# dogeplusplus/torch-actor-critic

Measured on AMD Instinct MI355X. Metric: sac_updates_per_sec, higher is better.
Workload: dtype bf16; 1 GPU; model=SAC-MLP[256, 256]-HalfCheetah-v4, global_batch=64, seq_len=1, parallelism=dp1, obs_dim=17, act_dim=6, replay_buffer=1000000, update_window=50, graph=True, engine=fused, mode=full

## Files before the change

### torch_actor_critic_amd/algo/act.py

```python

import numpy as np
import torch


class ActKernel:

    def __init__(self, actor, obs_dim: int, act_dim: int,
                 device: torch.device, philox_seed: int = 0):
        from ..models.mlp import Actor as MlpActor
        from ..ops import require_extension
        if type(actor) is not MlpActor:
            raise TypeError("ActKernel needs the plain MLP Actor")
        if any(l.out_features > 256 for l in actor.layers) or act_dim > 64:
            raise ValueError("shape outside act-kernel limits")
        self.ext = require_extension()
        self.ws = [l.weight for l in actor.layers]
        self.bs = [l.bias for l in actor.layers]
        self.wmu = actor.mu_layer.weight
        self.bmu = actor.mu_layer.bias
        self.wls = actor.log_std_layer.weight
        self.bls = actor.log_std_layer.bias
        self.act_limit = float(actor.act_limit)
        self.lo = float(actor.log_min_std)
        self.hi = float(actor.log_max_std)
        self.seed = philox_seed ^ 0x5ACB
        self.ctr = torch.zeros(1, dtype=torch.int64, device=device)
        self.obs_in = torch.zeros(obs_dim, device=device)
        self.obs_pin = torch.zeros(obs_dim, pin_memory=True)
        self.act_out = torch.zeros(act_dim, device=device)
        self.act_pin = torch.zeros(act_dim, pin_memory=True)
        self.flag_pin = torch.zeros(1, dtype=torch.int32, pin_memory=True)
        self.flag_np = self.flag_pin.numpy()
        self.ev = torch.cuda.Event()
        import os
        self._pinned_ok = os.environ.get("TAC_AMD_ACT_PINNED", "1") != "0"
        self._handle = self.ext.act_prepare(
            self.obs_pin, self.ws, self.bs, self.wmu, self.bmu, self.wls,
            self.bls, self.act_out, self.act_pin, self.flag_pin, self.ctr,
            self.seed, self.act_limit, self.lo, self.hi)

    def act(self, state: np.ndarray) -> np.ndarray:
        self.obs_pin.copy_(torch.from_numpy(np.asarray(state,
                                                       dtype=np.float32)))
        if self._pinned_ok:
            self.flag_pin[0] = 0
            self.ext.act_fire(self._handle)
            fl = self.flag_np
            for _ in range(2_000_000):
                if fl[0] != 0:
                    return self.act_pin.numpy().copy()
            torch.cuda.synchronize()
            if fl[0] != 0:
                return self.act_pin.numpy().copy()
            self._pinned_ok = False
        self.obs_in.copy_(self.obs_pin, non_blocking=True)
        self.ext.act_step(self.obs_in, self.ws, self.bs, self.wmu,
                          self.bmu, self.wls, self.bls, self.act_out,
                          self.ctr, self.seed, self.act_limit, self.lo,
                          self.hi)
        self.act_pin.copy_(self.act_out, non_blocking=True)
        self.ev.record()
        self.ev.synchronize()
        return self.act_pin.numpy().copy()


def make_act_path(actor, obs_dim, act_dim, device, philox_seed: int = 0):
    try:
        return ActKernel(actor, obs_dim, act_dim, device, philox_seed)
    except Exception:
        return ActGraph(actor, obs_dim, act_dim, device)


class BatchedActKernel:

    path = "kernel"
    MAX_LAYERS = 4
    MAX_OBS = 512

    def __init__(self, actor, obs_dim: int, act_dim: int, max_rows: int,
                 device: torch.device, philox_seed: int = 0):
        from ..models.mlp import Actor as MlpActor
        from ..ops import require_extension
        if type(actor) is not MlpActor:
            raise TypeError("BatchedActKernel needs the plain MLP Actor")
        if (any(l.out_features > 256 for l in actor.layers)
                or not 1 <= len(actor.layers) <= self.MAX_LAYERS
                or act_dim > 64 or obs_dim > self.MAX_OBS):
            raise ValueError("shape outside act-kernel limits")
        if torch.device(device).type != "cuda":
            raise ValueError("BatchedActKernel needs a cuda device")
        if max_rows < 1:
            raise ValueError("max_rows must be >= 1")
        self.ext = require_extension()
        self.actor = actor
        self.obs_dim = int(obs_dim)
        self.act_dim = int(act_dim)
        self.max_rows = int(max_rows)
        self.act_limit = float(actor.act_limit)
        self.lo = float(actor.log_min_std)
        self.hi = float(actor.log_max_std)
        self.seed = philox_seed ^ 0xE7A1
        self.ctr = 0
        self.obs_in = torch.zeros(max_rows, obs_dim, device=device)
        self.obs_pin = torch.zeros(max_rows, obs_dim, pin_memory=True)
        self.act_out = torch.zeros(max_rows, act_dim, device=device)
        self.act_pin = torch.zeros(max_rows, act_dim, pin_memory=True)
        self.ev = torch.cuda.Event()

    def launch(self, n: int, deterministic: bool, ctr: int):
        a = self.actor
        self.ext.act_batch(
            self.obs_in, [l.weight for l in a.layers],
            [l.bias for l in a.layers], a.mu_layer.weight, a.mu_layer.bias,
            a.log_std_layer.weight, a.log_std_layer.bias, self.act_out,
            n, bool(deterministic), int(ctr), self.seed, self.act_limit,
            self.lo, self.hi)

    def act(self, states, deterministic: bool = True) -> np.ndarray:
        s = np.asarray(states, dtype=np.float32).reshape(-1, self.obs_dim)
        n = s.shape[0]
        if not 1 <= n <= self.max_rows:
            raise ValueError(f"{n} states for max_rows={self.max_rows}")
        self.obs_pin[:n].copy_(torch.from_numpy(s))
        self.obs_in[:n].copy_(self.obs_pin[:n], non_blocking=True)
        if not deterministic:
            self.ctr += 1
# ... 172 lines not shown
```

### torch_actor_critic_amd/ops/csrc/fused.hip

```cpp

#include <hip/hip_runtime.h>
#include <hip/hip_bf16.h>

#include <torch/extension.h>
#include <c10/hip/HIPStream.h>

#include <algorithm>
#include <utility>
#include <vector>

#include "replay_draw.h"

namespace fused {

using namespace replay;

using f32x4 = __attribute__((ext_vector_type(4))) float;
using bf16x8 = __attribute__((ext_vector_type(8))) __bf16;

__global__ __launch_bounds__(256)
void philox_words2_kernel(int64_t* __restrict__ out, uint64_t seed,
                          uint64_t chi, uint64_t clo0, int64_t n) {
  philox_words_row(out, seed, chi, clo0, n);
}


struct MProb {
  const float* x; const float* w; const float* bias; float* y;
  const float* mask;
  const float* x2; const float* w2; const float* mask2;
  const float* r1_col;
  const float* r1_row;
};

constexpr int MAXZ = 4;

struct MGemm {
  MProb p[MAXZ];
  int M, N, K, lda, ldy;
  int K2;
  int nz, k_chunk;
  float* part;
};

constexpr int TB = 64;
constexpr int BKB2 = 64;
constexpr int BKF2 = 16;
constexpr int LDSB2 = 72;
constexpr int LDSF2 = 17;
constexpr int BKP = 128;
constexpr int LDSP = 136;

template <bool BF16, bool MASK>
DEVINL void stage_tile(void* lds, const float* src, const float* mask,
                       int r0, int k0, int R, int C, int ld) {
  const int tid = threadIdx.x;
  const int row = tid & 63;
  if constexpr (BF16) {
    __bf16* d = (__bf16*)lds;
    const int c0 = (tid >> 6) * 16;
    const int gr = r0 + row;
    bool interior = (r0 + 64 <= R) && (k0 + 64 <= C) && ((ld & 3) == 0)
                    && ((k0 & 3) == 0);
    if (interior) {
      const float* p = src + (int64_t)gr * ld + k0 + c0;
      float v[16];
#pragma unroll
      for (int q = 0; q < 4; ++q) {
        float4 f = *(const float4*)(p + q * 4);
        v[q * 4 + 0] = f.x; v[q * 4 + 1] = f.y;
        v[q * 4 + 2] = f.z; v[q * 4 + 3] = f.w;
      }
      if constexpr (MASK) {
        const float* mp = mask + (int64_t)gr * ld + k0 + c0;
#pragma unroll
        for (int q = 0; q < 4; ++q) {
          float4 f = *(const float4*)(mp + q * 4);
          v[q * 4 + 0] = f.x > 0.f ? v[q * 4 + 0] : 0.f;
          v[q * 4 + 1] = f.y > 0.f ? v[q * 4 + 1] : 0.f;
          v[q * 4 + 2] = f.z > 0.f ? v[q * 4 + 2] : 0.f;
          v[q * 4 + 3] = f.w > 0.f ? v[q * 4 + 3] : 0.f;
        }
      }
      union { __bf16 h[16]; uint4 u[2]; } pk;
#pragma unroll
      for (int e = 0; e < 16; ++e) pk.h[e] = (__bf16)v[e];
      uint4* dst = (uint4*)&d[row * LDSB2 + c0];
      dst[0] = pk.u[0];
      dst[1] = pk.u[1];
    } else {
#pragma unroll
      for (int e = 0; e < 16; ++e) {
        int c = c0 + e;
// ... 1803 lines not shown
      dy2_1[idx] = dqs[1][i] * wt3_1[j];
    }
  }
}


constexpr int ACT_MAXL = 4;
constexpr int ACT_MAXW = 512;

struct ActArgs {
  const float* x;
  const float* w[ACT_MAXL];
  const float* b[ACT_MAXL];
  int width[ACT_MAXL];
  int n_layers, O, A;
  const float* wmu; const float* bmu;
  const float* wls; const float* bls;
  float* action;
  int64_t* ctr;
  uint64_t seed;
  float act_limit, lo, hi;
};

struct ActPinned {
  float* out_host;
  int* flag_host;
};

__global__ __launch_bounds__(256)
void act_kernel(ActArgs a, ActPinned hp) {
  __shared__ __attribute__((aligned(16))) float buf[2][ACT_MAXW];
  __shared__ unsigned long long ctr_s;
  const int tid = threadIdx.x;
  if (tid == 0) ctr_s = (unsigned long long)(++a.ctr[0]);
  for (int k = tid; k < a.O; k += blockDim.x) buf[0][k] = a.x[k];
  __syncthreads();

  int cur = 0, K = a.O;
  for (int L = 0; L < a.n_layers; ++L) {
    const int H = a.width[L];
    float acc = 0.f;
    if (tid < H) {
      acc = a.b[L][tid];
      const float* wr = a.w[L] + (int64_t)tid * K;
      int k = 0;
      for (; k + 4 <= K; k += 4) {
        acc += wr[k] * buf[cur][k] + wr[k+1] * buf[cur][k+1]
             + wr[k+2] * buf[cur][k+2] + wr[k+3] * buf[cur][k+3];
      }
      for (; k < K; ++k) acc += wr[k] * buf[cur][k];
    }
    __syncthreads();
    if (tid < H) buf[1 - cur][tid] = fmaxf(acc, 0.f);
    __syncthreads();
    cur ^= 1;
    K = H;
  }

  if (tid < a.A) {
    float mu = a.bmu[tid], ls = a.bls[tid];
    const float* wm = a.wmu + (int64_t)tid * K;
    const float* wl = a.wls + (int64_t)tid * K;
    for (int k = 0; k < K; ++k) {
      float h = buf[cur][k];
      mu += wm[k] * h;
      ls += wl[k] * h;
    }
    ls = fminf(fmaxf(ls, a.lo), a.hi);
    Philox4 r = philox4(a.seed ^ 0x517cc1b727220a95ull, ctr_s, (uint64_t)tid);
    float eps = philox_normal(r.x, r.y);
    float act = tanhf(mu + expf(ls) * eps) * a.act_limit;
    a.action[tid] = act;
    if (hp.out_host) hp.out_host[tid] = act;
  }
  if (hp.flag_host) {
    __threadfence_system();
    __syncthreads();
    if (tid == 0) {
      __threadfence_system();
      *(volatile int*)hp.flag_host = 1;
    }
  }
}


constexpr int ACTB_R = 8;

__global__ __launch_bounds__(256)
void act_batch_kernel(ActArgs a, int N, int ldx, int deterministic,
                      unsigned long long ctr_val) {
  __shared__ __attribute__((aligned(16))) float buf[2][ACTB_R][ACT_MAXW];
  const int tid = threadIdx.x;
  const int row0 = blockIdx.x * ACTB_R;
  const int nrow = min(ACTB_R, N - row0);

  for (int i = tid; i < ACTB_R * a.O; i += blockDim.x) {
    const int r = i / a.O, k = i - r * a.O;
    buf[0][r][k] = r < nrow ? a.x[(int64_t)(row0 + r) * ldx + k] : 0.f;
  }
  __syncthreads();

  int cur = 0, K = a.O;
  for (int L = 0; L < a.n_layers; ++L) {
    const int H = a.width[L];
    float acc[ACTB_R];
    if (tid < H) {
      const float bias = a.b[L][tid];
#pragma unroll
      for (int r = 0; r < ACTB_R; ++r) acc[r] = bias;
      const float* wr = a.w[L] + (int64_t)tid * K;
      int k = 0;
      for (; k + 4 <= K; k += 4) {
        const float w0 = wr[k], w1 = wr[k+1], w2 = wr[k+2], w3 = wr[k+3];
#pragma unroll
        for (int r = 0; r < ACTB_R; ++r) {
          const float* h = &buf[cur][r][k];
          acc[r] += w0 * h[0] + w1 * h[1] + w2 * h[2] + w3 * h[3];
        }
      }
      for (; k < K; ++k) {
        const float w0 = wr[k];
#pragma unroll
        for (int r = 0; r < ACTB_R; ++r) acc[r] += w0 * buf[cur][r][k];
      }
#pragma unroll
      for (int r = 0; r < ACTB_R; ++r)
        buf[1 - cur][r][tid] = fmaxf(acc[r], 0.f);
    }
    __syncthreads();
    cur ^= 1;
    K = H;
  }

  if (tid < a.A) {
    float mu[ACTB_R], ls[ACTB_R];
    const float bm = a.bmu[tid];
    const float* wm = a.wmu + (int64_t)tid * K;
#pragma unroll
    for (int r = 0; r < ACTB_R; ++r) mu[r] = bm;
    if (deterministic) {
      for (int k = 0; k < K; ++k) {
        const float w = wm[k];
#pragma unroll
        for (int r = 0; r < ACTB_R; ++r) mu[r] += w * buf[cur][r][k];
      }
#pragma unroll
      for (int r = 0; r < ACTB_R; ++r)
        if (r < nrow)
          a.action[(int64_t)(row0 + r) * a.A + tid] =
              tanhf(mu[r]) * a.act_limit;
    } else {
      const float bl = a.bls[tid];
      const float* wl = a.wls + (int64_t)tid * K;
#pragma unroll
      for (int r = 0; r < ACTB_R; ++r) ls[r] = bl;
      for (int k = 0; k < K; ++k) {
        const float w = wm[k], v = wl[k];
#pragma unroll
        for (int r = 0; r < ACTB_R; ++r) {
          const float h = buf[cur][r][k];
          mu[r] += w * h;
          ls[r] += v * h;
        }
      }
#pragma unroll
      for (int r = 0; r < ACTB_R; ++r) {
// ... 1043 lines not shown
  need_vecM(logp, M, op, "logp");
  need_vecM(dq1, M, op, "dq1");
  need_vecM(dq2, M, op, "dq2");
  need_scalar_f32(loss_acc, op, "loss_acc");
  if (alpha_dev.has_value()) need_scalar_f32(*alpha_dev, op, "alpha_dev");
  if (mean_logp.has_value()) need_scalar_f32(*mean_logp, op, "mean_logp");
  LossFold lf{};
  lf.in.q1 = q1.data_ptr<float>();
  lf.in.q2 = q2.data_ptr<float>();
  lf.in.lpn = logp.data_ptr<float>();
  lf.alpha_dev = fptr(alpha_dev);
  lf.alpha_host = (float)alpha_host;
  lf.loss_acc = loss_acc.data_ptr<float>();
  lf.mean_logp = mean_logp.has_value() ? mean_logp->data_ptr<float>()
                                         : nullptr;
  lf.dq[0] = dq1.data_ptr<float>();
  lf.dq[1] = dq2.data_ptr<float>();
  launch_small_fold<1>(g, lf);
}

void adam_t(torch::Tensor p, torch::Tensor g, torch::Tensor m,
            torch::Tensor v, torch::Tensor step, double lr, double b1,
            double b2, double eps, double wd,
            std::vector<int64_t> offsets, std::vector<torch::Tensor> wts,
            c10::optional<torch::Tensor> targ, double rho,
            std::vector<int64_t> bss) {
  ATArgs ta{};
  ta.n_layers = (int)offsets.size();
  TORCH_CHECK(ta.n_layers <= MAX_T);
  TORCH_CHECK(wts.size() == offsets.size(),
              "adam_t: one W^T cache per slab offset");
  TORCH_CHECK(bss.empty() || bss.size() == offsets.size(),
              "adam_t: bss must be empty or hold one entry per slab");
  int64_t slab_end = 0;
  for (int i = 0; i < ta.n_layers; ++i) {
    TORCH_CHECK(offsets[i] >= slab_end,
                "adam_t: slab offsets must be strictly increasing and the "
                "slabs must not overlap (slab ", i, ")");
    slab_end = offsets[i] + wts[i].numel();
    TORCH_CHECK(wts[i].numel() > 0 && slab_end <= p.numel(),
                "adam_t: slab ", i, " does not lie inside [0, n)");
  }
  for (int i = 0; i < ta.n_layers; ++i) {
    ta.off[i] = offsets[i];
    ta.wt[i] = wts[i].data_ptr<float>();
    ta.BS[i] = bss.empty() ? 1 : (int)bss[i];
    TORCH_CHECK(wts[i].dim() == 2 && ta.BS[i] >= 1
                && wts[i].size(1) % ta.BS[i] == 0,
                "adam_t: W^T cache ", i, " must be [K, N * bs]");
    if (ta.BS[i] == 1) {
      ta.K[i] = (int)wts[i].size(0);
      ta.N[i] = (int)wts[i].size(1);
    } else {
      ta.K[i] = (int)wts[i].size(0);
      ta.N[i] = (int)(wts[i].size(1) / ta.BS[i]);
    }
  }
  int64_t n = p.numel();
  if (targ.has_value()) TORCH_CHECK(targ->numel() == n);
  int blocks = (int)std::min<int64_t>((n + 255) / 256, 1024);
  hipLaunchKernelGGL(adam_t_kernel, dim3(blocks), dim3(256), 0, stream(),
                     p.data_ptr<float>(), g.data_ptr<float>(),
                     m.data_ptr<float>(), v.data_ptr<float>(),
                     step.data_ptr<int64_t>(), n, (float)lr, (float)b1,
                     (float)b2, (float)eps, (float)wd,
                     targ.has_value() ? targ->data_ptr<float>() : nullptr,
                     (float)rho, ta);
}

torch::Tensor tg_eps(int64_t ctr_val, int64_t seed, int64_t R, int64_t A,
                     torch::Tensor like) {
  TORCH_CHECK(A >= 1 && A <= 64, "tg_eps: A = ", A,
              " outside 1..64 (one 64-lane block per row)");
  TORCH_CHECK(R >= 1 && R < (int64_t(1) << 31), "tg_eps: R must be >= 1");
  TORCH_CHECK(like.is_cuda() && like.scalar_type() == torch::kFloat32,
              "tg_eps: `like` must be an fp32 device tensor");
  auto out = torch::empty({R, A}, like.options());
  hipLaunchKernelGGL(tg_eps_kernel, dim3((int)R), dim3(64), 0, stream(),
                     out.data_ptr<float>(), (uint64_t)ctr_val,
                     (uint64_t)seed, (int)R, (int)A);
  return out;
}

void act_step(torch::Tensor x, std::vector<torch::Tensor> ws,
              std::vector<torch::Tensor> bs, torch::Tensor wmu,
              torch::Tensor bmu, torch::Tensor wls, torch::Tensor bls,
              torch::Tensor action, torch::Tensor ctr, int64_t seed,
              double act_limit, double lo, double hi) {
  ActArgs a{};
  a.n_layers = (int)ws.size();
  TORCH_CHECK(a.n_layers <= ACT_MAXL);
  a.x = x.data_ptr<float>();
  a.O = (int)x.numel();
  a.A = (int)action.numel();
  int maxw = a.O;
  for (int L = 0; L < a.n_layers; ++L) {
    a.w[L] = ws[L].data_ptr<float>();
    a.b[L] = bs[L].data_ptr<float>();
    a.width[L] = (int)ws[L].size(0);
    TORCH_CHECK(a.width[L] <= 256, "act kernel: trunk width > 256");
    maxw = std::max(maxw, a.width[L]);
  }
  TORCH_CHECK(maxw <= ACT_MAXW && a.A <= 256);
  a.wmu = wmu.data_ptr<float>();
  a.bmu = bmu.data_ptr<float>();
  a.wls = wls.data_ptr<float>();
  a.bls = bls.data_ptr<float>();
  a.action = action.data_ptr<float>();
  a.ctr = ctr.data_ptr<int64_t>();
  a.seed = (uint64_t)seed;
  a.act_limit = (float)act_limit;
  a.lo = (float)lo;
  a.hi = (float)hi;
  hipLaunchKernelGGL(act_kernel, dim3(1), dim3(256), 0, stream(), a,
                     ActPinned{nullptr, nullptr});
}

void act_step_pinned(torch::Tensor x, std::vector<torch::Tensor> ws,
                     std::vector<torch::Tensor> bs, torch::Tensor wmu,
                     torch::Tensor bmu, torch::Tensor wls,
                     torch::Tensor bls, torch::Tensor action,
                     torch::Tensor out_host, torch::Tensor flag_host,
                     torch::Tensor ctr, int64_t seed, double act_limit,
                     double lo, double hi) {
  TORCH_CHECK(out_host.is_pinned() && flag_host.is_pinned(),
              "host buffers must be pinned");
  ActArgs a{};
  a.n_layers = (int)ws.size();
  TORCH_CHECK(a.n_layers <= ACT_MAXL);
  a.x = x.data_ptr<float>();
  a.O = (int)x.numel();
  a.A = (int)action.numel();
  int maxw = a.O;
  for (int L = 0; L < a.n_layers; ++L) {
    a.w[L] = ws[L].data_ptr<float>();
    a.b[L] = bs[L].data_ptr<float>();
    a.width[L] = (int)ws[L].size(0);
    TORCH_CHECK(a.width[L] <= 256);
    maxw = std::max(maxw, a.width[L]);
  }
  TORCH_CHECK(maxw <= ACT_MAXW && a.A <= 256);
  a.wmu = wmu.data_ptr<float>();
  a.bmu = bmu.data_ptr<float>();
  a.wls = wls.data_ptr<float>();
  a.bls = bls.data_ptr<float>();
  a.action = action.data_ptr<float>();
  a.ctr = ctr.data_ptr<int64_t>();
  a.seed = (uint64_t)seed;
  a.act_limit = (float)act_limit;
  a.lo = (float)lo;
  a.hi = (float)hi;
  hipLaunchKernelGGL(act_kernel, dim3(1), dim3(256), 0, stream(), a,
                     ActPinned{out_host.data_ptr<float>(),
                               flag_host.data_ptr<int>()});
}

void bump3(torch::Tensor a, c10::optional<torch::Tensor> b,
           c10::optional<torch::Tensor> c) {
  hipLaunchKernelGGL(bump3_kernel, dim3(1), dim3(1), 0, stream(),
                     a.data_ptr<int64_t>(),
                     b.has_value() ? b->data_ptr<int64_t>() : nullptr,
                     c.has_value() ? c->data_ptr<int64_t>() : nullptr);
}

static std::vector<std::pair<ActArgs, ActPinned>> g_act_handles;

int64_t act_prepare(torch::Tensor x, std::vector<torch::Tensor> ws,
                    std::vector<torch::Tensor> bs, torch::Tensor wmu,
                    torch::Tensor bmu, torch::Tensor wls, torch::Tensor bls,
                    torch::Tensor action, torch::Tensor out_host,
                    torch::Tensor flag_host, torch::Tensor ctr,
                    int64_t seed, double act_limit, double lo, double hi) {
  TORCH_CHECK(out_host.is_pinned() && flag_host.is_pinned());
  ActArgs a{};
  a.n_layers = (int)ws.size();
  TORCH_CHECK(a.n_layers <= ACT_MAXL);
  a.x = x.data_ptr<float>();
  a.O = (int)x.numel();
  a.A = (int)action.numel();
  int maxw = a.O;
  for (int L = 0; L < a.n_layers; ++L) {
    a.w[L] = ws[L].data_ptr<float>();
    a.b[L] = bs[L].data_ptr<float>();
    a.width[L] = (int)ws[L].size(0);
    TORCH_CHECK(a.width[L] <= 256);
    maxw = std::max(maxw, a.width[L]);
  }
  TORCH_CHECK(maxw <= ACT_MAXW && a.A <= 256);
  a.wmu = wmu.data_ptr<float>();
  a.bmu = bmu.data_ptr<float>();
  a.wls = wls.data_ptr<float>();
  a.bls = bls.data_ptr<float>();
  a.action = action.data_ptr<float>();
  a.ctr = ctr.data_ptr<int64_t>();
  a.seed = (uint64_t)seed;
  a.act_limit = (float)act_limit;
  a.lo = (float)lo;
  a.hi = (float)hi;
  g_act_handles.push_back({a, ActPinned{out_host.data_ptr<float>(),
                                        flag_host.data_ptr<int>()}});
  return (int64_t)g_act_handles.size() - 1;
}

void act_fire(int64_t handle) {
  auto& h = g_act_handles.at((size_t)handle);
  hipLaunchKernelGGL(act_kernel, dim3(1), dim3(256), 0, stream(),
                     h.first, h.second);
}

void act_batch(torch::Tensor x, std::vector<torch::Tensor> ws,
               std::vector<torch::Tensor> bs, torch::Tensor wmu,
               torch::Tensor bmu, torch::Tensor wls, torch::Tensor bls,
               torch::Tensor action, int64_t n, bool deterministic,
               int64_t ctr_val, int64_t seed, double act_limit, double lo,
               double hi) {
  auto f32dev = [&](const torch::Tensor& t) {
    return t.is_cuda() && t.scalar_type() == torch::kFloat32
        && t.device() == x.device();
  };
  ActArgs a{};
  a.n_layers = (int)ws.size();
  TORCH_CHECK(a.n_layers >= 1 && a.n_layers <= ACT_MAXL
              && bs.size() == ws.size(), "act_batch: trunk depth");
  TORCH_CHECK(f32dev(x) && x.dim() == 2 && x.stride(1) == 1
              && x.stride(0) >= x.size(1), "act_batch: x must be [N, O] fp32 "
              "device rows");
  TORCH_CHECK(f32dev(action) && action.dim() == 2 && action.is_contiguous(),
              "act_batch: action must be contiguous [N, A] fp32");
  TORCH_CHECK(n >= 1 && n <= x.size(0) && n <= action.size(0),
              "act_batch: n outside the x/action buffers");
  a.x = x.data_ptr<float>();
  a.O = (int)x.size(1);
  a.A = (int)action.size(1);
  TORCH_CHECK(a.O >= 1 && a.O <= ACT_MAXW, "act_batch: obs width > ",
              ACT_MAXW);
  TORCH_CHECK(a.A >= 1 && a.A <= 64, "act_batch: act_dim > 64");
  int K = a.O;
  for (int L = 0; L < a.n_layers; ++L) {
    TORCH_CHECK(f32dev(ws[L]) && ws[L].is_contiguous() && ws[L].dim() == 2
                && ws[L].size(1) == K, "act_batch: trunk weight ", L);
    a.width[L] = (int)ws[L].size(0);
    TORCH_CHECK(a.width[L] >= 1 && a.width[L] <= 256,
                "act_batch: trunk width > 256");
    TORCH_CHECK(f32dev(bs[L]) && bs[L].is_contiguous()
                && bs[L].numel() == a.width[L], "act_batch: trunk bias ", L);
    a.w[L] = ws[L].data_ptr<float>();
    a.b[L] = bs[L].data_ptr<float>();
    K = a.width[L];
  }
  for (const torch::Tensor* w : {&wmu, &wls})
    TORCH_CHECK(f32dev(*w) && w->is_contiguous() && w->dim() == 2
                && w->size(0) == a.A && w->size(1) == K,
                "act_batch: head weight");
  for (const torch::Tensor* b : {&bmu, &bls})
    TORCH_CHECK(f32dev(*b) && b->is_contiguous() && b->numel() == a.A,
                "act_batch: head bias");
  a.wmu = wmu.data_ptr<float>();
  a.bmu = bmu.data_ptr<float>();
  a.wls = wls.data_ptr<float>();
  a.bls = bls.data_ptr<float>();
  a.action = action.data_ptr<float>();
  a.ctr = nullptr;
  a.seed = (uint64_t)seed;
  a.act_limit = (float)act_limit;
  a.lo = (float)lo;
  a.hi = (float)hi;
  const int grid = (int)((n + ACTB_R - 1) / ACTB_R);
  hipLaunchKernelGGL(act_batch_kernel, dim3(grid), dim3(256), 0, stream(),
                     a, (int)n, (int)x.stride(0), deterministic ? 1 : 0,
                     (unsigned long long)ctr_val);
}

torch::Tensor philox_words2(int64_t seed, int64_t chi, int64_t clo0,
                            int64_t n) {
  TORCH_CHECK(n >= 1 && n <= (int64_t(1) << 20),
              "philox_words2: n outside 1..2^20");
  auto out = torch::empty({n, 4}, torch::dtype(torch::kInt64)
                                      .device(torch::kCUDA));
  hipLaunchKernelGGL(philox_words2_kernel, dim3((int)((n + 255) / 256)),
                     dim3(256), 0, stream(), out.data_ptr<int64_t>(),
                     (uint64_t)seed, (uint64_t)chi, (uint64_t)clo0, n);
  return out;
}

void alpha_update(torch::Tensor log_alpha, torch::Tensor alpha_dev,
                  torch::Tensor m, torch::Tensor v, torch::Tensor step,
                  torch::Tensor mean_logp, double target_entropy, double lr) {
  need_scalar_f32(log_alpha, "alpha_update", "log_alpha");
  need_scalar_f32(alpha_dev, "alpha_update", "alpha_dev");
  need_scalar_f32(m, "alpha_update", "m");
// ... 12 lines not shown
void register_fused(pybind11::module_& m) {
  m.def("mgemm", &fused::mgemm,
        "multi-problem MFMA GEMM (fwd-form, strided, masked, sum2)");
  m.def("mgemm_r1", &fused::mgemm_r1,
        "masked GEMM whose A operand is a rank-1 product formed on read");
  m.def("mgemm_r1_qloss", &fused::mgemm_r1_qloss,
        "qloss2 + K=1 dgrad + masked dgrad in one small-shape launch");
  m.def("mgemm_r1_piloss", &fused::mgemm_r1_piloss,
        "piloss2 + mgemm_r1 in one small-shape launch");
  m.def("mgemm_r1_fold_ok", &fused::mgemm_r1_fold_ok,
        "host-only: do (M, K) pass the gate of the two folded entries");
  m.def("mgemm_small_mode", &fused::mgemm_small_mode,
        "set TAC_AMD_MGEMM_SMALL's mode (0 = pipelined kernel only), "
        "returns the previous mode");
  m.def("mwgrad", &fused::mwgrad, "multi-problem wgrad + fused db");
  m.def("mwgrad_het", &fused::mwgrad_het,
        "heterogeneous multi-problem wgrad: one launch per phase");
  m.def("mwgrad_het_adam", &fused::mwgrad_het_adam,
        "heterogeneous wgrad with Adam (+polyak, +W^T) in the epilogue");
  m.def("mwgrad_het_adam_split", &fused::mwgrad_het_adam_split,
        "host-only: M slabs mwgrad_het_adam would use for these shapes");
  m.def("ranges_tile_exactly", &fused::ranges_tile_exactly,
        "host-only: do [off, off+len) ranges tile [0, n) exactly once");
  m.def("transpose_multi", &fused::transpose_multi,
        pybind11::arg("ws"), pybind11::arg("wts"),
        pybind11::arg("blocks") = std::vector<int64_t>{});
  namespace py = pybind11;
  m.def("gather2", &fused::gather2, py::arg("state"), py::arg("act"),
        py::arg("rew"), py::arg("nstate"), py::arg("done"),
        py::arg("size_dev"), py::arg("ctr"), py::arg("seed"), py::arg("xc"),
        py::arg("xc2"), py::arg("orew"), py::arg("od"), py::arg("B"),
        py::arg("ctr_add") = 0);
  m.def("gather2n", &fused::gather2n, py::arg("state"), py::arg("act"),
        py::arg("rew"), py::arg("nstate"), py::arg("done"),
        py::arg("ep_end"), py::arg("size_dev"), py::arg("ptr_dev"),
        py::arg("ctr"), py::arg("seed"), py::arg("n"), py::arg("gamma"),
        py::arg("xc"), py::arg("xc2"), py::arg("orew"), py::arg("od"),
        py::arg("B"), py::arg("ctr_add") = 0);
  m.def("gather2p", &fused::gather2p, py::arg("state"), py::arg("act"),
        py::arg("rew"), py::arg("nstate"), py::arg("done"),
        py::arg("ep_end"), py::arg("size_dev"), py::arg("ptr_dev"),
        py::arg("tree"), py::arg("ctr"), py::arg("seed"), py::arg("n"),
        py::arg("gamma"), py::arg("xc"), py::arg("xc2"), py::arg("orew"),
        py::arg("od"), py::arg("idx_out"), py::arg("prob_out"),
        py::arg("u_out"), py::arg("B"), py::arg("ctr_add") = 0);
  m.def("per_update", &fused::per_update,
        "sum tree: leaves[idx] = (td + eps)^alpha, ancestors recomputed");
  m.def("per_set_range", &fused::per_set_range,
        "sum tree: a ring range gets max_priority, ancestors recomputed");
  m.def("tg_fwd2", &fused::tg_fwd2, py::arg("hl"), py::arg("out0"),
        py::arg("col0"), py::arg("out1"), py::arg("col1"), py::arg("B0"),
        py::arg("logp"), py::arg("prob"), py::arg("ctr"), py::arg("seed"),
        py::arg("act_limit"), py::arg("lo"), py::arg("hi"),
        py::arg("ctr_add") = 0);
  m.def("tg_bwd2", &fused::tg_bwd2);
  m.def("qloss2", &fused::qloss2, py::arg("q1"), py::arg("q2"),
        py::arg("q1t"), py::arg("q2t"), py::arg("logp_next"),
        py::arg("rew"), py::arg("done"), py::arg("alpha_dev"),
        py::arg("alpha_host"), py::arg("loss_acc"), py::arg("dq1"),
        py::arg("dq2"), py::arg("B"), py::arg("gamma"), py::arg("scale"),
        py::arg("wt3_0"), py::arg("wt3_1"), py::arg("dy2_0"),
        py::arg("dy2_1"), py::arg("h2"), py::arg("bump0") = py::none(),
        py::arg("bump1") = py::none(), py::arg("bump2") = py::none(),
        py::arg("prob") = py::none(), py::arg("size_dev") = py::none(),
        py::arg("beta_dev") = py::none(), py::arg("td") = py::none());
  m.def("piloss2", &fused::piloss2);
  m.def("alpha_update", &fused::alpha_update);
  m.def("tg_eps", &fused::tg_eps);
  m.def("philox_words2", &fused::philox_words2,
        "test helper: raw Philox words of this translation unit's copy");
  m.def("adam_t", &fused::adam_t,
        pybind11::arg("p"), pybind11::arg("g"), pybind11::arg("m"),
        pybind11::arg("v"), pybind11::arg("step"), pybind11::arg("lr"),
        pybind11::arg("b1"), pybind11::arg("b2"), pybind11::arg("eps"),
        pybind11::arg("wd"), pybind11::arg("offsets"),
        pybind11::arg("wts"), pybind11::arg("targ"),
        pybind11::arg("rho"),
        pybind11::arg("bss") = std::vector<int64_t>{});
  m.def("act_step", &fused::act_step);
  m.def("bump3", &fused::bump3);
  m.def("act_step_pinned", &fused::act_step_pinned);
  m.def("act_prepare", &fused::act_prepare);
  m.def("act_fire", &fused::act_fire);
  m.def("act_batch", &fused::act_batch,
        "batched actor forward (deterministic or Philox-stochastic)");
}
```

Before: 7029 updates/s.

## Add latency-shaped single-state actor kernel and fused C++ launch-and-spin act path

Adds act_fast_kernel, which front-loads all weight, bias and head loads into registers and prefetches layer weights in 64-wide K slabs with double-buffered register staging into LDS, so the single-state actor forward is not a chain of serial global-memory round trips. It also adds act_sync, a C++ entry point that copies the observation into pinned memory, launches the kernel and spins on the pinned flag with a CPU pause and timeout, which removes Python-level torch copies and polling from each environment step. The cost is a second kernel with a strict shape gate and fallback logic, environment-variable switches, and a changed fp contraction and summation order that may shift results slightly.

New measurement: 7378 updates/s, median of 6. 1.05x the previous value.

```diff
diff --git a/torch_actor_critic_amd/algo/act.py b/torch_actor_critic_amd/algo/act.py
--- a/torch_actor_critic_amd/algo/act.py
+++ b/torch_actor_critic_amd/algo/act.py
@@ -34,14 +34,26 @@
         self.ev = torch.cuda.Event()
         import os
         self._pinned_ok = os.environ.get("TAC_AMD_ACT_PINNED", "1") != "0"
+        self._sync = os.environ.get("TAC_AMD_ACT_SYNC", "1") != "0"
+        self.obs_dim, self.act_dim = int(obs_dim), int(act_dim)
         self._handle = self.ext.act_prepare(
             self.obs_pin, self.ws, self.bs, self.wmu, self.bmu, self.wls,
             self.bls, self.act_out, self.act_pin, self.flag_pin, self.ctr,
             self.seed, self.act_limit, self.lo, self.hi)
 
     def act(self, state: np.ndarray) -> np.ndarray:
-        self.obs_pin.copy_(torch.from_numpy(np.asarray(state,
-                                                       dtype=np.float32)))
+        if self._pinned_ok and self._sync:
+            obs = np.ascontiguousarray(state, dtype=np.float32).reshape(-1)
+            out = np.empty(self.act_dim, dtype=np.float32)
+            if self.ext.act_sync(self._handle, obs, out):
+                return out
+            torch.cuda.synchronize()
+            if self.flag_np[0] != 0:
+                return self.act_pin.numpy().copy()
+            self._pinned_ok = False
+        else:
+            self.obs_pin.copy_(torch.from_numpy(
+                np.asarray(state, dtype=np.float32)))
         if self._pinned_ok:
             self.flag_pin[0] = 0
             self.ext.act_fire(self._handle)
diff --git a/torch_actor_critic_amd/ops/csrc/act_sync.h b/torch_actor_critic_amd/ops/csrc/act_sync.h
--- /dev/null
+++ b/torch_actor_critic_amd/ops/csrc/act_sync.h
@@ -0,0 +1,40 @@
+#pragma once
+
+#include <chrono>
+#include <cstring>
+
+namespace actsync {
+
+constexpr double kTimeoutS = 0.1;
+
+inline void cpu_pause() {
+#if defined(__x86_64__) || defined(__i386__)
+  __builtin_ia32_pause();
+#elif defined(__aarch64__)
+  asm volatile("yield");
+#endif
+}
+
+template <class Launch>
+inline bool run(float* obs_pin, const float* obs, int n_obs,
+                const float* act_pin, float* out, int n_act, int* flag,
+                double timeout_s, Launch&& launch) {
+  std::memcpy(obs_pin, obs, sizeof(float) * (size_t)n_obs);
+  __atomic_store_n(flag, 0, __ATOMIC_RELEASE);
+  launch();
+  using clock = std::chrono::steady_clock;
+  const auto t0 = clock::now();
+  for (;;) {
+    for (int i = 0; i < 64; ++i) {
+      if (__atomic_load_n(flag, __ATOMIC_ACQUIRE) != 0) {
+        std::memcpy(out, act_pin, sizeof(float) * (size_t)n_act);
+        return true;
+      }
+      cpu_pause();
+    }
+    if (std::chrono::duration<double>(clock::now() - t0).count() > timeout_s)
+      return false;
+  }
+}
+
+}
diff --git a/torch_actor_critic_amd/ops/csrc/fused.hip b/torch_actor_critic_amd/ops/csrc/fused.hip
--- a/torch_actor_critic_amd/ops/csrc/fused.hip
+++ b/torch_actor_critic_amd/ops/csrc/fused.hip
@@ -4,11 +4,14 @@
 
 #include <torch/extension.h>
 #include <c10/hip/HIPStream.h>
+#include <pybind11/numpy.h>
 
 #include <algorithm>
+#include <cstdint>
 #include <utility>
 #include <vector>
 
+#include "act_sync.h"
 #include "replay_draw.h"
 
 namespace fused {
@@ -1978,6 +1981,239 @@
     }
   }
 }
+
+
+constexpr int ACTF_L0 = 36;
+constexpr int ACTF_KS = 64;
+constexpr int ACTF_SV = ACTF_KS / 4;
+constexpr int ACTF_SS = ACTF_KS + 4;
+constexpr int ACTF_HV = 8;
+constexpr int ACTF_HL = 2 * ACTF_HV * 256 + 128 * 4;
+
+struct ActfLds {
+  float act[2][256];
+  float bias[ACT_MAXL][256];
+  float w0[ACTF_L0 * 256];
+  float slab[256 * ACTF_SS];
+  float hd[ACTF_HL];
+  float ls[64];
+  unsigned long long ctr;
+};
+
+struct ActfCur {
+  int L, k0, K, H;
+  const float* w;
+};
+
+DEVINL void actf_shape(const ActArgs& a, ActfCur& c) {
+  c.K = c.L == 1 ? a.width[0] : c.L == 2 ? a.width[1] : a.width[2];
+  c.H = c.L == 1 ? a.width[1] : c.L == 2 ? a.width[2] : a.width[3];
+  c.w = c.L == 1 ? a.w[1] : c.L == 2 ? a.w[2] : a.w[3];
+}
+
+DEVINL ActfCur actf_next(const ActArgs& a, ActfCur c) {
+  if (c.L < a.n_layers) {
+    c.k0 += ACTF_KS;
+    if (c.k0 >= c.K) { ++c.L; c.k0 = 0; actf_shape(a, c); }
+  }
+  return c;
+}
+
+template <bool FULL>
+DEVINL void actf_issue(f32x4 (&R)[ACTF_SV], const ActfCur& cu, int tid) {
+  const unsigned vo = (unsigned)(tid >> 4) * cu.K + (tid & 15) * 4;
+#pragma unroll
+  for (int j = 0; j < ACTF_SV; ++j) {
+    if (FULL || 16 * j < cu.H) {
+      const float* p = cu.w + cu.k0 + (int64_t)(16 * j) * cu.K;
+      R[j] = *reinterpret_cast<const f32x4*>(p + vo);
+    }
+  }
+}
+
+template <bool FULL>
+DEVINL void actf_commit(const f32x4 (&R)[ACTF_SV], float* slab,
+                        const ActfCur& cu, int tid) {
+  float* d = slab + (tid >> 4) * ACTF_SS + (tid & 15) * 4;
+#pragma unroll
+  for (int j = 0; j < ACTF_SV; ++j)
+    if (FULL || 16 * j < cu.H)
+      *reinterpret_cast<f32x4*>(d + 16 * j * ACTF_SS) = R[j];
+}
+
+__global__ __launch_bounds__(256)
+void act_fast_kernel(ActArgs a, ActPinned hp) {
+#pragma clang fp contract(off)
+  __shared__ __attribute__((aligned(16))) ActfLds s;
+  const int tid = threadIdx.x;
+  const int O = a.O, A = a.A, nl = a.n_layers;
+  const int H0 = a.width[0];
+  const int KL = nl == 1 ? a.width[0] : nl == 2 ? a.width[1]
+               : nl == 3 ? a.width[2] : a.width[3];
+
+  const float xo = a.x[tid < O ? tid : 0];
+  const long long c_old = a.ctr[0];
+  float br[ACT_MAXL];
+#pragma unroll
+  for (int L = 0; L < ACT_MAXL; ++L)
+    br[L] = L < nl ? a.b[L][tid < a.width[L] ? tid : 0] : 0.f;
+  const int hl = tid & 63;
+  const bool h_on = tid < 128 && hl < A;
+  float hv = (tid < 64 ? a.bmu : a.bls)[hl < A ? hl : 0];
+
+  float v0[ACTF_L0];
+  const int n0 = H0 * O;
+  const int r0 = (n0 + 255) >> 8;
+#pragma unroll
+  for (int g = 0; g < ACTF_L0 / 6; ++g) {
+    if (6 * g < r0) {
+#pragma unroll
+      for (int j = 6 * g; j < 6 * g + 6; ++j)
+        v0[j] = a.w[0][min(tid + 256 * j, n0 - 1)];
+    }
+  }
+
+  f32x4 RA[ACTF_SV], RB[ACTF_SV];
+  ActfCur cu{1, 0, 0, 0, nullptr};
+  actf_shape(a, cu);
+  auto issue = [&](f32x4 (&R)[ACTF_SV], const ActfCur& c) {
+    if (c.L < nl) {
+      if (c.H == 256) actf_issue<true>(R, c, tid);
+      else actf_issue<false>(R, c, tid);
+    }
+  };
+  issue(RA, cu);
+  issue(RB, actf_next(a, cu));
+
+  float hm[ACTF_HV], hs[ACTF_HV];
+  const int nh = A * KL;
+  const int rh = (nh + 255) >> 8;
+#pragma unroll
+  for (int g = 0; g < ACTF_HV / 4; ++g) {
+    if (4 * g < rh) {
+#pragma unroll
+      for (int j = 4 * g; j < 4 * g + 4; ++j) {
+        const int idx = min(tid + 256 * j, nh - 1);
+        hm[j] = a.wmu[idx];
+        hs[j] = a.wls[idx];
+      }
+    }
+  }
+
+  if (tid < O) s.act[0][tid] = xo;
+#pragma unroll
+  for (int L = 0; L < ACT_MAXL; ++L) s.bias[L][tid] = br[L];
+  if (tid == 0) {
+    const long long c_new = c_old + 1;
+    a.ctr[0] = c_new;
+    s.ctr = (unsigned long long)c_new;
+  }
+#pragma unroll
+  for (int g = 0; g < ACTF_L0 / 6; ++g) {
+    if (6 * g < r0) {
+#pragma unroll
+      for (int j = 6 * g; j < 6 * g + 6; ++j)
+        s.w0[min(tid + 256 * j, n0 - 1)] = v0[j];
+    }
+  }
+  __syncthreads();
+
+  int cur = 1;
+  {
+    float acc = br[0];
+    if (tid < H0) {
+      const float* wr = s.w0 + tid * O;
+      const float* x = s.act[0];
+      int k = 0;
+      for (; k + 4 <= O; k += 4)
+        acc += wr[k] * x[k] + wr[k+1] * x[k+1]
+             + wr[k+2] * x[k+2] + wr[k+3] * x[k+3];
+      for (; k < O; ++k) acc = __builtin_fmaf(wr[k], x[k], acc);
+      s.act[1][tid] = fmaxf(acc, 0.f);
+    }
+  }
+
+  float acc = br[1];
+  auto slab_step = [&](f32x4 (&R)[ACTF_SV]) {
+    if (cu.H == 256) actf_commit<true>(R, s.slab, cu, tid);
+    else actf_commit<false>(R, s.slab, cu, tid);
+    __syncthreads();
+    issue(R, actf_next(a, actf_next(a, cu)));
+    if (tid < cu.H) {
+      const f32x4* wr = reinterpret_cast<const f32x4*>(s.slab + tid * ACTF_SS);
+      const f32x4* x = reinterpret_cast<const f32x4*>(s.act[cur] + cu.k0);
+#pragma unroll
+      for (int g = 0; g < ACTF_SV; ++g) {
+        const f32x4 w = wr[g], h = x[g];
+        acc += w.x * h.x + w.y * h.y + w.z * h.z + w.w * h.w;
+      }
+    }
+    if (cu.k0 + ACTF_KS >= cu.K) {
+      if (tid < cu.H) s.act[1 - cur][tid] = fmaxf(acc, 0.f);
+      cur ^= 1;
+      acc = s.bias[cu.L + 1 < ACT_MAXL ? cu.L + 1 : 0][tid];
+    }
+    __syncthreads();
+    cu = actf_next(a, cu);
+  };
+  while (cu.L < nl) {
+    slab_step(RA);
+    if (cu.L >= nl) break;
+    slab_step(RB);
+  }
+
+  const int HS = KL + 4;
+  {
+    const int sh = 31 - __builtin_clz(KL);
+    float* hd_ls = s.hd + A * HS;
+#pragma unroll
+    for (int g = 0; g < ACTF_HV / 4; ++g) {
+      if (4 * g < rh) {
+#pragma unroll
+        for (int j = 4 * g; j < 4 * g + 4; ++j) {
+          const int idx = min(tid + 256 * j, nh - 1);
+          const int d = (idx >> sh) * HS + (idx & (KL - 1));
+          s.hd[d] = hm[j];
+          hd_ls[d] = hs[j];
+        }
+      }
+    }
+  }
+  __syncthreads();
+  if (h_on) {
+    const int row = tid < 64 ? hl : A + hl;
+    const f32x4* wr = reinterpret_cast<const f32x4*>(s.hd + row * HS);
+    const f32x4* x = reinterpret_cast<const f32x4*>(s.act[cur]);
+    for (int g = 0; g < (KL >> 2); ++g) {
+      const f32x4 w = wr[g], h = x[g];
+      hv = __builtin_fmaf(w.x, h.x, hv);
+      hv = __builtin_fmaf(w.y, h.y, hv);
+      hv = __builtin_fmaf(w.z, h.z, hv);
+      hv = __builtin_fmaf(w.w, h.w, hv);
+    }
+    if (tid >= 64) s.ls[hl] = hv;
+  }
+  __syncthreads();
+  if (tid < A) {
+    const float mu = hv;
+    float ls = s.ls[tid];
+    ls = fminf(fmaxf(ls, a.lo), a.hi);
+    Philox4 r = philox4(a.seed ^ 0x517cc1b727220a95ull, s.ctr, (uint64_t)tid);
+    float eps = philox_normal(r.x, r.y);
+    float act = tanhf(__builtin_fmaf(expf(ls), eps, mu)) * a.act_limit;
+    a.action[tid] = act;
+    if (hp.out_host) hp.out_host[tid] = act;
+  }
+  if (hp.flag_host) {
+    __threadfence_system();
+    __syncthreads();
+    if (tid == 0) {
+      __threadfence_system();
+      *(volatile int*)hp.flag_host = 1;
+    }
+  }
+}
+
 
 
 constexpr int ACTB_R = 8;
@@ -3187,11 +3423,14 @@
   return out;
 }
 
-void act_step(torch::Tensor x, std::vector<torch::Tensor> ws,
-              std::vector<torch::Tensor> bs, torch::Tensor wmu,
-              torch::Tensor bmu, torch::Tensor wls, torch::Tensor bls,
-              torch::Tensor action, torch::Tensor ctr, int64_t seed,
-              double act_limit, double lo, double hi) {
+static ActArgs act_args(const torch::Tensor& x,
+                        const std::vector<torch::Tensor>& ws,
+                        const std::vector<torch::Tensor>& bs,
+                        const torch::Tensor& wmu, const torch::Tensor& bmu,
+                        const torch::Tensor& wls, const torch::Tensor& bls,
+                        const torch::Tensor& action,
+                        const torch::Tensor& ctr, int64_t seed,
+                        double act_limit, double lo, double hi) {
   ActArgs a{};
   a.n_layers = (int)ws.size();
   TORCH_CHECK(a.n_layers <= ACT_MAXL);
@@ -3217,8 +3456,82 @@
   a.act_limit = (float)act_limit;
   a.lo = (float)lo;
   a.hi = (float)hi;
-  hipLaunchKernelGGL(act_kernel, dim3(1), dim3(256), 0, stream(), a,
-                     ActPinned{nullptr, nullptr});
+  return a;
+}
+
+static int g_act_fast = -1;
+
+static bool act_fast_mode_get() {
+  if (g_act_fast < 0) {
+    const char* e = getenv("TAC_AMD_ACT_FAST");
+    g_act_fast = e ? (atoi(e) != 0) : 1;
+  }
+  return g_act_fast != 0;
+}
+
+int64_t act_fast_mode(int64_t mode) {
+  const int prev = act_fast_mode_get();
+  TORCH_CHECK(mode == 0 || mode == 1, "act_fast_mode: 0 or 1");
+  g_act_fast = (int)mode;
+  return prev;
+}
+
+static bool act_fast_shape_ok(int O, const int* width, int n_layers, int A) {
+  if (n_layers < 1 || n_layers > ACT_MAXL) return false;
+  if (O < 1 || O > 256 || A < 1 || A > 64) return false;
+  for (int L = 0; L < n_layers; ++L)
+    if (width[L] < 4 || width[L] > 256 || width[L] % 4 != 0) return false;
+  for (int L = 1; L < n_layers; ++L)
+    if (width[L - 1] % ACTF_KS != 0 || width[L] % 16 != 0) return false;
+  const int KL = width[n_layers - 1];
+  if ((KL & (KL - 1)) != 0) return false;
+  if ((int64_t)width[0] * O > ACTF_L0 * 256) return false;
+  if ((int64_t)A * KL > ACTF_HV * 256) return false;
+  return true;
+}
+
+bool act_fast_ok(int64_t obs_dim, std::vector<int64_t> widths,
+                 int64_t act_dim) {
+  if (widths.empty() || widths.size() > (size_t)ACT_MAXL) return false;
+  if (obs_dim < 1 || obs_dim > 256 || act_dim < 1 || act_dim > 64)
+    return false;
+  int w[ACT_MAXL] = {};
+  for (size_t L = 0; L < widths.size(); ++L) {
+    if (widths[L] < 1 || widths[L] > 256) return false;
+    w[L] = (int)widths[L];
+  }
+  return act_fast_shape_ok((int)obs_dim, w, (int)widths.size(),
+                           (int)act_dim);
+}
+
+static bool act_fast_fits(const ActArgs& a) {
+  if (!act_fast_shape_ok(a.O, a.width, a.n_layers, a.A)) return false;
+  for (int L = 1; L < a.n_layers; ++L)
+    if (reinterpret_cast<uintptr_t>(a.w[L]) % 16 != 0) return false;
+  return true;
+}
+
+static bool g_act_last_fast = false;
+
+static void act_launch(const ActArgs& a, const ActPinned& hp, bool fits) {
+  g_act_last_fast = fits && act_fast_mode_get();
+  if (g_act_last_fast)
+    hipLaunchKernelGGL(act_fast_kernel, dim3(1), dim3(256), 0, stream(), a,
+                       hp);
+  else
+    hipLaunchKernelGGL(act_kernel, dim3(1), dim3(256), 0, stream(), a, hp);
+}
+
+bool act_last_fast() { return g_act_last_fast; }
+
+void act_step(torch::Tensor x, std::vector<torch::Tensor> ws,
+              std::vector<torch::Tensor> bs, torch::Tensor wmu,
+              torch::Tensor bmu, torch::Tensor wls, torch::Tensor bls,
+              torch::Tensor action, torch::Tensor ctr, int64_t seed,
+              double act_limit, double lo, double hi) {
+  const ActArgs a = act_args(x, ws, bs, wmu, bmu, wls, bls, action, ctr,
+                             seed, act_limit, lo, hi);
+  act_launch(a, ActPinned{nullptr, nullptr}, act_fast_fits(a));
 }
 
 void act_step_pinned(torch::Tensor x, std::vector<torch::Tensor> ws,
@@ -3230,34 +3543,10 @@
                      double lo, double hi) {
   TORCH_CHECK(out_host.is_pinned() && flag_host.is_pinned(),
               "host buffers must be pinned");
-  ActArgs a{};
-  a.n_layers = (int)ws.size();
-  TORCH_CHECK(a.n_layers <= ACT_MAXL);
-  a.x = x.data_ptr<float>();
-  a.O = (int)x.numel();
-  a.A = (int)action.numel();
-  int maxw = a.O;
-  for (int L = 0; L < a.n_layers; ++L) {
-    a.w[L] = ws[L].data_ptr<float>();
-    a.b[L] = bs[L].data_ptr<float>();
-    a.width[L] = (int)ws[L].size(0);
-    TORCH_CHECK(a.width[L] <= 256);
-    maxw = std::max(maxw, a.width[L]);
-  }
-  TORCH_CHECK(maxw <= ACT_MAXW && a.A <= 256);
-  a.wmu = wmu.data_ptr<float>();
-  a.bmu = bmu.data_ptr<float>();
-  a.wls = wls.data_ptr<float>();
-  a.bls = bls.data_ptr<float>();
-  a.action = action.data_ptr<float>();
-  a.ctr = ctr.data_ptr<int64_t>();
-  a.seed = (uint64_t)seed;
-  a.act_limit = (float)act_limit;
-  a.lo = (float)lo;
-  a.hi = (float)hi;
-  hipLaunchKernelGGL(act_kernel, dim3(1), dim3(256), 0, stream(), a,
-                     ActPinned{out_host.data_ptr<float>(),
-                               flag_host.data_ptr<int>()});
+  const ActArgs a = act_args(x, ws, bs, wmu, bmu, wls, bls, action, ctr,
+                             seed, act_limit, lo, hi);
+  act_launch(a, ActPinned{out_host.data_ptr<float>(),
+                          flag_host.data_ptr<int>()}, act_fast_fits(a));
 }
 
 void bump3(torch::Tensor a, c10::optional<torch::Tensor> b,
@@ -3268,7 +3557,13 @@
                      c.has_value() ? c->data_ptr<int64_t>() : nullptr);
 }
 
-static std::vector<std::pair<ActArgs, ActPinned>> g_act_handles;
+struct ActHandle {
+  ActArgs a;
+  ActPinned hp;
+  bool fits;
+  bool x_pinned;
+};
+static std::vector<ActHandle> g_act_handles;
 
 int64_t act_prepare(torch::Tensor x, std::vector<torch::Tensor> ws,
                     std::vector<torch::Tensor> bs, torch::Tensor wmu,
@@ -3277,40 +3572,42 @@
                     torch::Tensor flag_host, torch::Tensor ctr,
                     int64_t seed, double act_limit, double lo, double hi) {
   TORCH_CHECK(out_host.is_pinned() && flag_host.is_pinned());
-  ActArgs a{};
-  a.n_layers = (int)ws.size();
-  TORCH_CHECK(a.n_layers <= ACT_MAXL);
-  a.x = x.data_ptr<float>();
-  a.O = (int)x.numel();
-  a.A = (int)action.numel();
-  int maxw = a.O;
-  for (int L = 0; L < a.n_layers; ++L) {
-    a.w[L] = ws[L].data_ptr<float>();
-    a.b[L] = bs[L].data_ptr<float>();
-    a.width[L] = (int)ws[L].size(0);
-    TORCH_CHECK(a.width[L] <= 256);
-    maxw = std::max(maxw, a.width[L]);
-  }
-  TORCH_CHECK(maxw <= ACT_MAXW && a.A <= 256);
-  a.wmu = wmu.data_ptr<float>();
-  a.bmu = bmu.data_ptr<float>();
-  a.wls = wls.data_ptr<float>();
-  a.bls = bls.data_ptr<float>();
-  a.action = action.data_ptr<float>();
-  a.ctr = ctr.data_ptr<int64_t>();
-  a.seed = (uint64_t)seed;
-  a.act_limit = (float)act_limit;
-  a.lo = (float)lo;
-  a.hi = (float)hi;
+  TORCH_CHECK(out_host.numel() == action.numel() && flag_host.numel() >= 1);
+  const ActArgs a = act_args(x, ws, bs, wmu, bmu, wls, bls, action, ctr,
+                             seed, act_limit, lo, hi);
   g_act_handles.push_back({a, ActPinned{out_host.data_ptr<float>(),
-                                        flag_host.data_ptr<int>()}});
+                                        flag_host.data_ptr<int>()},
+                           act_fast_fits(a), x.is_pinned()});
   return (int64_t)g_act_handles.size() - 1;
 }
 
 void act_fire(int64_t handle) {
   auto& h = g_act_handles.at((size_t)handle);
-  hipLaunchKernelGGL(act_kernel, dim3(1), dim3(256), 0, stream(),
-                     h.first, h.second);
+  act_launch(h.a, h.hp, h.fits);
+}
+
+bool act_handle_fast(int64_t handle) {
+  return g_act_handles.at((size_t)handle).fits && act_fast_mode_get();
+}
+
+bool act_sync(int64_t handle, py::array obs, py::array out) {
+  auto& h = g_act_handles.at((size_t)handle);
+  TORCH_CHECK(h.x_pinned, "act_sync: the handle's observation buffer is "
+              "not pinned host memory");
+  auto f32vec = [](const py::array& v, int n) {
+    return py::isinstance<py::array_t<float>>(v) && v.ndim() == 1
+        && v.shape(0) == n && v.strides(0) == (py::ssize_t)sizeof(float);
+  };
+  TORCH_CHECK(f32vec(obs, h.a.O), "act_sync: obs must be a contiguous "
+              "float32 array of length ", h.a.O);
+  TORCH_CHECK(f32vec(out, h.a.A) && out.writeable(), "act_sync: out must "
+              "be a writeable contiguous float32 array of length ", h.a.A);
+  return actsync::run(const_cast<float*>(h.a.x),
+                       static_cast<const float*>(obs.data()), h.a.O,
+                       h.hp.out_host,
+                       static_cast<float*>(out.mutable_data()), h.a.A,
+                       h.hp.flag_host, actsync::kTimeoutS,
+                       [&] { act_launch(h.a, h.hp, h.fits); });
 }
 
 void act_batch(torch::Tensor x, std::vector<torch::Tensor> ws,
@@ -3489,6 +3786,18 @@
   m.def("act_step_pinned", &fused::act_step_pinned);
   m.def("act_prepare", &fused::act_prepare);
   m.def("act_fire", &fused::act_fire);
+  m.def("act_sync", &fused::act_sync,
+        "act_fire + host spin in one call: (handle, obs, out) -> landed");
+  m.def("act_fast_ok", &fused::act_fast_ok,
+        "host-only: do (obs_dim, trunk widths, act_dim) pass the shape "
+        "gate of the latency-shaped act kernel");
+  m.def("act_fast_mode", &fused::act_fast_mode,
+        "set TAC_AMD_ACT_FAST's mode (0 = act_kernel only), returns the "
+        "previous mode");
+  m.def("act_handle_fast", &fused::act_handle_fast,
+        "host-only: would act_fire(handle) launch the latency-shaped form");
+  m.def("act_last_fast", &fused::act_last_fast,
+        "host-only: did the last single-state act launch use it");
   m.def("act_batch", &fused::act_batch,
         "batched actor forward (deterministic or Philox-stochastic)");
 }
```
